# tjiangHIT/cuteSV

Hardware: NVIDIA H100
Metric: sv_signatures_clustered_per_sec (higher is better)
Workload: dtype int32

## Files before the change

### cutesv_b200/csrc/cutesv_b200.cu

```cuda
#include <cuda_runtime.h>
#include <dlfcn.h>
#include <nccl.h>
#include <stdarg.h>
#include <stdio.h>
#include <stdlib.h>
#include <string.h>

#include <algorithm>
#include <atomic>
#include <string>
#include <vector>

#include "../../include/cutesv_b200.h"
#include "core.h"
#include "devprims.cuh"
#include "host_tables.h"
#include "kernels.cuh"
#include "radix.cuh"
#include "extract.cuh"
#include "scan_core.h"

using namespace csv;

static thread_local char g_err[1024] = "";
// ... 109 lines not shown
struct LbPool {
    uint32_t* tickets = nullptr;
    const uint32_t* epoch = nullptr;
    uint32_t ord0 = 0;
    int next = 0, cap = 0;
};

struct GcWork {
    DBuf win, bin_base, bin_start, bin_fill, bin_list, iter, prim, cov_off, ovl_off, cov_fill, ovl_fill, cov_u, ovl_u, lb, words;
    DBuf r_chrom, r_start, r_end, r_id, r_prim, cov_raw, ovl_raw, cov_ded, ovl_ded, cov_flag, ovl_flag, sup_off, sup, geno;
    uint32_t n_cov = 0, n_ovl = 0;
};

struct SsWork {
    DBuf keys_a, keys_b, vals_a, vals_b, keep, tie, kchrom, order, off, hist, lb, words;
};

struct csv_ctx {
    int device = 0;
    cudaStream_t stream = nullptr;
    bool own_stream = false;
    cudaStream_t copy_stream = nullptr;
    cudaEvent_t ev_up[CSV_NTYPES + 1] = {nullptr, nullptr, nullptr, nullptr, nullptr, nullptr};
    bool up_pending[CSV_NTYPES + 1] = {false, false, false, false, false, false};
    bool up_device[CSV_NTYPES + 1] = {false, false, false, false, false, false};
    bool up_checked[CSV_NTYPES + 1] = {false, false, false, false, false, false};
    DBuf up_status;
    cudaEvent_t ev_prod = nullptr;
    cudaEvent_t ev_done = nullptr;
    bool done_pending = false;
    int n_sm = 132;
    csv_params P;
    bool have_params = false;
    int32_t n_contigs = 0;
    std::vector<int64_t> contig_len;
    std::vector<uint64_t> contig_off;
    int64_t off_pad = 0;
    std::vector<uint8_t> owned;
    DBuf d_off, d_len, d_len_eff;
    SigBuf sig[CSV_NTYPES];
    int64_t n_reads = 0;
    DBuf r_chrom, r_start, r_end, r_id, r_prim;
    int64_t n_aln = 0;
    DBuf a_chrom, a_start, a_end, a_id, a_prim, a_off, a_span;
    DBuf tickets, scan_carry, emit_cursor;
    DBuf d_epoch;
    LbPool lb;
    uint32_t epoch_host = 0;
    bool small_chain[CSV_NTYPES] = {false, false, false, false, false};
    bool prefilter_enabled = true;
    bool records_enabled = true;
    bool small_path_enabled = true;
    int64_t pair_cap_override = 0;
    DBuf d_goff[CSV_NTYPES + 1];
    Lane lanes[N_LANES];
    cudaEvent_t ev_fork = nullptr;
    cudaStream_t side_stream[2] = {nullptr, nullptr};
    cudaEvent_t ev_side_fork[2] = {nullptr, nullptr}, ev_side_join[2] = {nullptr, nullptr};
    cudaStream_t aux_stream = nullptr;
    cudaEvent_t ev_aux = nullptr;
    bool lanes_enabled = true;
    DBuf kept[CSV_NTYPES], cnt;
    uint32_t kept_cap[CSV_NTYPES] = {0, 0, 0, 0, 0};
    DBuf cand_tmp, cand, geno, names, counters;
    uint32_t cap_cand = 0, cap_names = 0;
    Counters* h_counters = nullptr;
    DBuf bin_start, bin_fill, bin_bits, win_list, win_rec, dr, has_rows, gl_table, pow_half, pairs;
    uint32_t pow_n = 0;
    bool ran = false, counts_valid = false;
    int64_t launches = 0;
    bool profiling = false;
    bool lane_marks = false;
    struct Interval { int st; cudaEvent_t a, b; int64_t bytes; };
    std::vector<Interval> ivs;
    std::vector<cudaEvent_t> ev_pool;
    size_t ev_next = 0;
    bool ivs_consumed = false;
    struct KInterval { const char* name; cudaEvent_t a, b; };
    std::vector<KInterval> kivs;
    struct KTotal { std::string name; int64_t launches; double ms; };
    std::vector<KTotal> ktotals;
    float stage_ms[CSV_ST_COUNT];
    float sort_ms = 0.f;
    int64_t sort_bytes = 0;
    int32_t sort_launches = 0;
    uint32_t last_mask = 0x1f;
    ExtractState ex;
    struct GraphKey {
        uint32_t mask; int64_t n[CSV_NTYPES]; int64_t n_reads, n_aln; csv_params P; int lanes; uint64_t alloc_epoch; uint64_t cfg_epoch;
        bool small_chain[CSV_NTYPES];
        bool up_checked[CSV_NTYPES + 1];
    };
    struct GraphSlot { bool valid = false; GraphKey key; cudaGraphExec_t exec = nullptr; int64_t launches = 0; uint64_t used = 0; };
    static constexpr int N_GRAPHS = 4;
    GraphSlot graphs[N_GRAPHS];
    GraphKey last_key;
    bool last_key_valid = false;
    bool graphs_enabled = true;
    uint64_t cfg_epoch = 1, graph_clock = 0;
    int64_t graph_replays = 0;
    struct P2PState {
        bool ready = false, failed = false;
        void* box = nullptr;
        int64_t slot_bytes = 0;
        size_t flags_off = 0;
        std::vector<void*> peer;
        DBuf d_tab;
        unsigned long long epoch = 0;
    } p2p;
    bool p2p_enabled = true;
    ncclComm_t comm = nullptr;
    int rank = 0, world = 1;
    DBuf g_send, g_recv, g_cand, g_geno, g_names, g_scratch, g_tab;
// ... 137 lines not shown
    CU(c->gl_table.ensure(gl.size() * sizeof(csv_geno)));
    CU(cudaMemcpy(c->gl_table.p, gl.data(), gl.size() * sizeof(csv_geno), cudaMemcpyHostToDevice));
    std::vector<double> ph = build_pow_half(pow_n);
    CU(c->pow_half.ensure(ph.size() * sizeof(double)));
    CU(cudaMemcpy(c->pow_half.p, ph.data(), ph.size() * sizeof(double), cudaMemcpyHostToDevice));
    c->pow_n = pow_n;
    return CSV_OK;
}

extern "C" int csv_create(int device, void* stream, csv_ctx** out) {
    if (!out) return set_err(CSV_E_INVALID, "null out");
    int n_dev = 0;
    cudaError_t e = cudaGetDeviceCount(&n_dev);
    if (e != cudaSuccess || n_dev == 0)
        return set_err(CSV_E_NODEVICE, "no CUDA device (%s): cutesv_b200 has no CPU fallback",
                       e == cudaSuccess ? "device count 0" : cudaGetErrorString(e));
    if (device < 0 || device >= n_dev) return set_err(CSV_E_INVALID, "device %d out of range (%d devices)", device, n_dev);
    cudaDeviceProp prop;
    CU(cudaGetDeviceProperties(&prop, device));
    if (prop.major != 9 || prop.minor != 0)
        return set_err(CSV_E_NODEVICE, "device %d is sm_%d%d; this library is built for sm_90a only", device, prop.major, prop.minor);
    CU(cudaSetDevice(device));
    csv_ctx* c = new csv_ctx();
    c->device = device;
    c->n_sm = prop.multiProcessorCount;
    if (stream) { c->stream = (cudaStream_t)stream; c->own_stream = false; }
    else {
        cudaError_t e2 = cudaStreamCreateWithFlags(&c->stream, cudaStreamNonBlocking);
        if (e2 != cudaSuccess) { delete c; return set_err(CSV_E_CUDA, "cudaStreamCreate: %s", cudaGetErrorString(e2)); }
        c->own_stream = true;
    }
    c->lanes[0].stream = c->stream;
    {
        cudaError_t e4 = cudaStreamCreateWithFlags(&c->copy_stream, cudaStreamNonBlocking);
        for (int i = 0; i <= CSV_NTYPES && e4 == cudaSuccess; i++) e4 = cudaEventCreateWithFlags(&c->ev_up[i], cudaEventDisableTiming);
        if (e4 == cudaSuccess) e4 = cudaEventCreateWithFlags(&c->ev_done, cudaEventDisableTiming);
        if (e4 == cudaSuccess) e4 = cudaEventCreateWithFlags(&c->ev_prod, cudaEventDisableTiming);
        if (e4 == cudaSuccess) e4 = cudaEventCreateWithFlags(&c->ev_fork, cudaEventDisableTiming);
        if (e4 == cudaSuccess) e4 = cudaStreamCreateWithFlags(&c->aux_stream, cudaStreamNonBlocking);
        if (e4 == cudaSuccess) e4 = cudaEventCreateWithFlags(&c->ev_aux, cudaEventDisableTiming);
        for (int k = 0; k < 2 && e4 == cudaSuccess; k++) {
            e4 = cudaStreamCreateWithFlags(&c->side_stream[k], cudaStreamNonBlocking);
            if (e4 == cudaSuccess) e4 = cudaEventCreateWithFlags(&c->ev_side_fork[k], cudaEventDisableTiming);
            if (e4 == cudaSuccess) e4 = cudaEventCreateWithFlags(&c->ev_side_join[k], cudaEventDisableTiming);
        }
        for (int l = 1; l < N_LANES && e4 == cudaSuccess; l++) {
            e4 = cudaStreamCreateWithFlags(&c->lanes[l].stream, cudaStreamNonBlocking);
            if (e4 == cudaSuccess) e4 = cudaEventCreateWithFlags(&c->lanes[l].ev_join, cudaEventDisableTiming);
        }
        if (e4 != cudaSuccess) { delete c; return set_err(CSV_E_CUDA, "copy stream / lanes: %s", cudaGetErrorString(e4)); }
    }
    csv_default_params(&c->P);
    if (const char* e = getenv("CUTESV_B200_PAIR_CAP")) c->pair_cap_override = atoll(e);
    if (const char* e = getenv("CUTESV_B200_NO_PREFILTER")) c->prefilter_enabled = atoi(e) == 0;
    if (const char* e = getenv("CUTESV_B200_LANES")) c->lanes_enabled = atoi(e) != 0;
    if (const char* e = getenv("CUTESV_B200_GRAPHS")) c->graphs_enabled = atoi(e) != 0;
    if (const char* e = getenv("CUTESV_B200_PDL")) c->pdl_enabled = atoi(e) != 0;
    if (const char* e = getenv("CUTESV_B200_GATHER")) c->p2p_enabled = strcmp(e, "nccl") != 0;
    if (const char* e = getenv("CUTESV_B200_RECORDS")) c->records_enabled = atoi(e) != 0;
    if (const char* e = getenv("CUTESV_B200_SMALL_PATH")) c->small_path_enabled = atoi(e) != 0;
    if (const char* e = getenv("CUTESV_B200_SMALL_CHAIN")) for (int t = 0; t < CSV_NTYPES; t++) c->small_chain[t] = atoi(e) != 0;
    for (int s = 0; s < CSV_ST_COUNT; s++) c->stage_ms[s] = 0.f;
    cudaError_t e3 = cudaMallocHost((void**)&c->h_counters, sizeof(Counters));
    if (e3 != cudaSuccess) { delete c; return set_err(CSV_E_CUDA, "cudaMallocHost: %s", cudaGetErrorString(e3)); }
    int rc = upload_tables(c, 1u << 16);
    if (rc != CSV_OK) { delete c; return rc; }
    CU(c->d_epoch.ensure(64, true));
    CU(c->emit_cursor.ensure(256, true));
    CU(c->up_status.ensure((CSV_NTYPES + 1) * 4, true));
    const int smem_warp = (CL_THREADS / 32) * WARP_M * ARENA_PER_MAX + (CL_THREADS / 32) * 40 * 8;
    CU(cudaFuncSetAttribute(k_cluster_warp<0>, cudaFuncAttributeMaxDynamicSharedMemorySize, smem_warp));
    CU(cudaFuncSetAttribute(k_cluster_warp<1>, cudaFuncAttributeMaxDynamicSharedMemorySize, smem_warp));
    CU(cudaFuncSetAttribute(k_cluster_warp<2>, cudaFuncAttributeMaxDynamicSharedMemorySize, smem_warp));
    CU(cudaFuncSetAttribute(k_cluster_warp<3>, cudaFuncAttributeMaxDynamicSharedMemorySize, smem_warp));
    CU(cudaFuncSetAttribute(k_cluster_warp<4>, cudaFuncAttributeMaxDynamicSharedMemorySize, smem_warp));
    CU(cudaFuncSetAttribute(k_cluster_warp<5>, cudaFuncAttributeMaxDynamicSharedMemorySize, smem_warp));
    CU(cudaFuncSetAttribute(k_cluster_warp<6>, cudaFuncAttributeMaxDynamicSharedMemorySize, smem_warp));
    CU(cudaFuncSetAttribute(k_cluster_warp<7>, cudaFuncAttributeMaxDynamicSharedMemorySize, smem_warp));
    CU(cudaFuncSetAttribute(k_cluster_block<0>, cudaFuncAttributeMaxDynamicSharedMemorySize, BLOCK_M * ARENA_PER_MAX));
    CU(cudaFuncSetAttribute(k_cluster_block<1>, cudaFuncAttributeMaxDynamicSharedMemorySize, BLOCK_M * ARENA_PER_MAX));
    CU(cudaFuncSetAttribute(k_cluster_block<2>, cudaFuncAttributeMaxDynamicSharedMemorySize, BLOCK_M * ARENA_PER_MAX));
    CU(cudaFuncSetAttribute(k_cluster_block<3>, cudaFuncAttributeMaxDynamicSharedMemorySize, BLOCK_M * ARENA_PER_MAX));
    CU(cudaFuncSetAttribute(k_part_filter, cudaFuncAttributeMaxDynamicSharedMemorySize, (int)pf_smem_bytes(PART_W_MAX)));
    CU(cudaFuncSetAttribute(k_part_scatter, cudaFuncAttributeMaxDynamicSharedMemorySize, (int)ps_smem_bytes()));
    *out = c;
    return CSV_OK;
}

extern "C" int csv_destroy(csv_ctx* c) {
    if (!c) return CSV_OK;
    cudaSetDevice(c->device);
    cudaStreamSynchronize(c->stream);
    for (auto& g : c->graphs) if (g.exec) cudaGraphExecDestroy(g.exec);
    if (c->comm) comm_destroy(c);
    if (c->h_gather) cudaFreeHost(c->h_gather);
    for (int l = 1; l < N_LANES; l++) {
        Lane& L = c->lanes[l];
        if (L.stream) { cudaStreamSynchronize(L.stream); cudaStreamDestroy(L.stream); }
        if (L.ev_join) cudaEventDestroy(L.ev_join);
    }
    if (c->ev_fork) cudaEventDestroy(c->ev_fork);
    if (c->aux_stream) { cudaStreamSynchronize(c->aux_stream); cudaStreamDestroy(c->aux_stream); }
    if (c->ev_aux) cudaEventDestroy(c->ev_aux);
    for (int k = 0; k < 2; k++) {
        if (c->side_stream[k]) { cudaStreamSynchronize(c->side_stream[k]); cudaStreamDestroy(c->side_stream[k]); }
        if (c->ev_side_fork[k]) cudaEventDestroy(c->ev_side_fork[k]);
// ... 668 lines not shown
    J.sv.chrom = w.u_chrom.as<int32_t>(); J.sv.a = w.u_a.as<int32_t>(); J.sv.b = w.u_b.as<int32_t>();
    J.sv.rid = w.u_rid.as<int32_t>(); J.sv.c = w.u_c.as<int32_t>();
    return run_segment_and_cluster(c, L, J, t, kslot_base);
}

static int ensure_small(Lane& L, size_t ns) {
    SmallWork& w = L.small;
    CU(w.k_rid.ensure(ns * 4)); CU(w.k_b.ensure(ns * 4)); CU(w.k_prim.ensure(ns * 8)); CU(w.perm_a.ensure(ns * 4)); CU(w.perm_b.ensure(ns * 4));
    CU(w.sel.ensure(ns * 4)); CU(w.u_chrom.ensure(ns * 4)); CU(w.u_a.ensure(ns * 4)); CU(w.u_b.ensure(ns * 4)); CU(w.u_rid.ensure(ns * 4));
    CU(w.u_c.ensure(ns * 4));
    return CSV_OK;
}
static int ensure_lane_scratch(Lane& L, size_t nm) {
    CU(L.keys_a.ensure(nm * 8)); CU(L.keys_b.ensure(nm * 8)); CU(L.vals_a.ensure(nm * 4)); CU(L.vals_b.ensure(nm * 4));
    CU(L.big_list.ensure((nm / WARP_M + 2) * 4));
    CU(L.giant_list.ensure((nm / BLOCK_M + 2) * 4));
    CU(L.giant_arena.ensure(nm * 2 * ARENA_PER_MAX + 256));
    return CSV_OK;
}

static int ensure_workspace(csv_ctx* c, uint32_t type_mask) {
    int64_t n_max = 0, n_total = 0, n_small_max = 0;
    for (int t = 0; t < CSV_NTYPES; t++) {
        if (!(type_mask >> t & 1)) continue;
        n_max = std::max(n_max, c->sig[t].n);
        n_total += c->sig[t].n;
        if (t >= CSV_INV) n_small_max = std::max(n_small_max, c->sig[t].n);
    }
    const size_t nm = (size_t)std::max<int64_t>(n_max, 1);
    int rc = ensure_lane_scratch(c->lanes[0], nm);
    if (rc) return rc;
    if (c->lanes_enabled) {
        for (int t = 1; t < CSV_NTYPES; t++) {
            const int64_t nl = (type_mask >> t & 1) ? c->sig[t].n : 0;
            if (nl == 0) continue;
            if ((rc = ensure_lane_scratch(c->lanes[t], (size_t)nl))) return rc;
            if (t >= CSV_INV && (rc = ensure_small(c->lanes[t], (size_t)nl))) return rc;
        }
    }
    CU(c->tickets.ensure(LB_ORDINALS * 4));
    CU(c->counters.ensure(sizeof(Counters)));
    if ((rc = ensure_small(c->lanes[0], (size_t)std::max<int64_t>(n_small_max, 1)))) return rc;
    uint64_t kept_total = 0;
    const int ms = std::max(1, c->P.min_support);
    for (int t = 0; t < CSV_NTYPES; t++) {
        if (!(type_mask >> t & 1)) continue;
        c->kept_cap[t] = (uint32_t)(c->sig[t].n / ms + 1);
        CU(c->kept[t].ensure((size_t)c->kept_cap[t] * 4));
        kept_total += c->kept_cap[t];
    }
    CU(c->cnt.ensure((size_t)kept_total * 4 + 4));
    const int ms_a = std::max(1, std::min(c->P.min_support, std::max(1, c->P.min_support_allele)));
    c->cap_cand = (uint32_t)(2 * (n_total / ms_a) + 16);
    c->cap_names = (uint32_t)(n_total + 16);
    CU(c->cand_tmp.ensure((size_t)c->cap_cand * sizeof(csv_cand)));
    CU(c->cand.ensure((size_t)c->cap_cand * sizeof(csv_cand)));
    CU(c->geno.ensure((size_t)c->cap_cand * sizeof(csv_geno)));
    CU(c->names.ensure((size_t)c->cap_names * 4));
    CU(c->dr.ensure((size_t)c->cap_cand * 4));
    CU(c->win_list.ensure((size_t)c->cap_cand * 2 * 4));
    CU(c->win_rec.ensure((size_t)c->cap_cand * 2 * sizeof(WinRec)));
    CU(c->has_rows.ensure((size_t)c->n_contigs + 16));
    return CSV_OK;
}

static int join_lanes(csv_ctx* c) {
    for (int l = 1; l < N_LANES; l++) {
        Lane& L = c->lanes[l];
        if (!L.used) continue;
        CU(cudaEventRecord(L.ev_join, L.stream));
        CU(cudaStreamWaitEvent(c->stream, L.ev_join, 0));
        L.used = false;
    }
    return CSV_OK;
}

static int enqueue_cluster(csv_ctx* c, uint32_t type_mask) {
    int rc;
    stage_reset_if_consumed(c);
    c->last_mask = type_mask;
    c->lb = LbPool{c->tickets.as<uint32_t>(), c->d_epoch.as<uint32_t>(), 0, 0, (int)LB_ORDINALS};
    {
        int n_lanes = 0;
        for (int t = 0; t < CSV_NTYPES; t++) n_lanes += ((type_mask >> t & 1) && c->sig[t].n > 0) ? 1 : 0;
        c->pdl_now = c->pdl_enabled && n_lanes <= 2;
    }
    LAUNCH(c, c->stream, k_begin, 1, 256, 0, c->d_epoch.as<uint32_t>(), c->tickets.as<uint32_t>(), (int)LB_ORDINALS, c->counters.as<uint32_t>(),
           (int)(sizeof(Counters) / 4), c->emit_cursor.as<unsigned long long>());
    Counters* ctr = c->counters.as<Counters>();
    uint32_t kslot_base = 0;
    const bool lanes = c->lanes_enabled;
    if (lanes) CU(cudaEventRecord(c->ev_fork, c->stream));
    for (Lane& L : c->lanes) L.used = false;
    const uint64_t total_len = c->contig_off[c->n_contigs];
    int geno_shift = 10;
    while ((total_len >> geno_shift) > (1u << 20)) geno_shift++;
    const uint32_t geno_bins = (uint32_t)(total_len >> geno_shift) + 2;
    bool aux_used = false;
    if (c->P.genotype) {
        CU(c->bin_start.ensure(((size_t)geno_bins + 1) * 4));
        CU(c->bin_fill.ensure((size_t)geno_bins * 4));
        CU(c->bin_bits.ensure(((size_t)geno_bins / 32 + 2) * 4));
        cudaStream_t rs = lanes ? c->aux_stream : c->stream;
        if (lanes) CU(cudaStreamWaitEvent(rs, c->ev_fork, 0));
        CU(cudaMemsetAsync(c->bin_start.p, 0, ((size_t)geno_bins + 1) * 4, rs));
        CU(cudaMemsetAsync(c->bin_fill.p, 0, (size_t)geno_bins * 4, rs));
        CU(cudaMemsetAsync(c->bin_bits.p, 0, ((size_t)geno_bins / 32 + 2) * 4, rs));
        CU(cudaMemsetAsync(c->has_rows.p, 0, (size_t)c->n_contigs, rs));
        if (lanes) { CU(cudaEventRecord(c->ev_aux, rs)); aux_used = true; }
    }
    for (int t = 0; t < CSV_NTYPES; t++) {
        if (!(type_mask >> t & 1) || c->sig[t].n == 0) continue;
        Lane& L = c->lanes[lanes ? t : 0];
        if (&L != &c->lanes[0] && !L.used) { CU(cudaStreamWaitEvent(L.stream, c->ev_fork, 0)); L.used = true; }
        rc = wait_upload(c, L.stream, t);
        if (!rc && c->up_checked[t]) LAUNCH(c, L.stream, k_fold_status, 1, 32, 0, c->up_status.as<uint32_t>() + t, &ctr->status);
        if (!rc) rc = (t == CSV_DEL || t == CSV_INS) ? run_indel(c, L, t, kslot_base) : run_other(c, L, t, kslot_base);
        if (rc) {
            join_lanes(c);
            if (aux_used) cudaStreamWaitEvent(c->stream, c->ev_aux, 0);
            return rc;
        }
        kslot_base += c->kept_cap[t];
    }
    rc = join_lanes(c);
    if (rc) return rc;
    if (aux_used) CU(cudaStreamWaitEvent(c->stream, c->ev_aux, 0));
    int tail_mark = -1;
    if (c->lane_marks) { kprof_begin(c, c->stream, "tail"); tail_mark = (int)c->kivs.size() - 1; }
    GenoJob G;
    memset(&G, 0, sizeof(G));
    G.cand = c->cand.as<csv_cand>(); G.geno = c->geno.as<csv_geno>(); G.names = c->names.as<int32_t>(); G.ctr = ctr;
    G.cap_cand = c->cap_cand;
    G.ct = ContigTab{c->d_off.as<uint64_t>(), c->d_len_eff.as<int64_t>(), c->n_contigs};
    G.gp = GtParams{c->P.bias_del, c->P.gt_bias_ins, c->P.bias_dup, c->P.bias_inv};
    G.shift = geno_shift;
    G.n_bins = geno_bins;
    G.bin_start = c->bin_start.as<uint32_t>(); G.bin_fill = c->bin_fill.as<uint32_t>(); G.bin_bits = c->bin_bits.as<uint32_t>();
    G.win_list = c->win_list.as<uint32_t>(); G.win_cap = c->cap_cand * 2;
    G.lin32 = (total_len + 4096) < (1ull << 32) ? 1 : 0;
    G.win_rec = c->win_rec.as<WinRec>();
    G.dr = c->dr.as<uint32_t>(); G.has_rows = c->has_rows.as<uint8_t>();
    G.gl_table = c->gl_table.as<csv_geno>();
    G.genotype = c->P.genotype;
    stage_begin(c, c->stream, CSV_ST_ORDER);
    {
        CU(c->scan_carry.ensure(64));
        uint32_t* carry = c->scan_carry.as<uint32_t>();
        uint32_t kb = 0;
        int prev = -1;
        for (int t = 0; t < CSV_NTYPES; t++) {
            if (!(type_mask >> t & 1) || c->sig[t].n == 0) continue;
            TileSync ts;
            rc = make_sync(c->lb, c->lanes[0].lb_status, c->stream, (size_t)(c->kept_cap[t] / SEL_TILE + 2), &ts);
            if (rc) return rc;
            if (prev >= 0)
                LAUNCH_PDL(c, c->stream, (k_scan_excl<8>), grid_for(c, std::max<int64_t>(c->kept_cap[t], 1), SEL_TILE, 2), SEL_THREADS, 0, c->cnt.as<uint32_t>() + kb,
                           (int64_t)c->kept_cap[t], (const uint32_t*)&ctr->n_kept[t], (const uint32_t*)(carry + prev), carry + t, ts);
            else
                LAUNCH(c, c->stream, (k_scan_excl<8>), grid_for(c, std::max<int64_t>(c->kept_cap[t], 1), SEL_TILE, 2), SEL_THREADS, 0, c->cnt.as<uint32_t>() + kb,
                       (int64_t)c->kept_cap[t], (const uint32_t*)&ctr->n_kept[t], (const uint32_t*)nullptr, carry + t, ts);
            kb += c->kept_cap[t];
            prev = t;
        }
        LAUNCH_PDL(c, c->stream, k_permute, grid_for(c, c->cap_cand, 256, 4), 256, 0, c->cand_tmp.as<csv_cand>(), c->cnt.as<uint32_t>(), ctr, c->cap_cand,
               c->cand.as<csv_cand>(), G, c->emit_cursor.as<unsigned long long>());
    }
    stage_end(c, c->stream, CSV_ST_ORDER);
    rc = wait_upload(c, c->stream, CSV_NTYPES);
    if (rc) return rc;
    if (c->up_checked[CSV_NTYPES] && c->n_reads > 0)
        LAUNCH(c, c->stream, k_fold_status, 1, 32, 0, c->up_status.as<uint32_t>() + CSV_NTYPES, &ctr->status);
    stage_begin(c, c->stream, CSV_ST_GENOTYPE);
    {
        if (c->P.genotype) {
            TileSync ts;
            rc = make_sync(c->lb, c->lanes[0].lb_status, c->stream, (size_t)((G.n_bins + 1) / (SEL_THREADS * 4) + 2), &ts);
            if (rc) return rc;
            LAUNCH_PDL(c, c->stream, (k_scan_excl<4>), grid_for(c, G.n_bins + 1, SEL_THREADS * 4, 4), SEL_THREADS, 0, G.bin_start, (int64_t)G.n_bins + 1,
                   (const uint32_t*)nullptr, (const uint32_t*)nullptr, (uint32_t*)nullptr, ts);
            LAUNCH_PDL(c, c->stream, (k_windows<1>), grid_for(c, c->cap_cand, 256, 4), 256, 0, G);
            if (c->n_reads > 0) {
                PairBuf PB;
                PB.cap = (uint32_t)std::min<int64_t>(4 * c->n_reads + (1 << 20), (int64_t)1 << 30);
                if (c->pair_cap_override > 0) PB.cap = (uint32_t)c->pair_cap_override;
                CU(c->pairs.ensure((size_t)PB.cap * (G.lin32 ? sizeof(uint4) : sizeof(uint2))));
                PB.pairs = c->pairs.as<uint2>();
                PB.pairs4 = c->pairs.as<uint4>();
                PB.count = &ctr->n_windows;
                if (G.lin32) {
                    LAUNCH_PDL(c, c->stream, (k_reads_pass<true>), std::min(grid_for(c, c->n_reads, 1024, 8), resident_grid(c, k_reads_pass<true>, 256, 0)), 256, 0, G, PB, c->r_chrom.as<int32_t>(), c->r_start.as<int32_t>(),
                           c->r_end.as<int32_t>(), c->r_id.as<int32_t>(), c->r_prim.as<uint8_t>(), c->n_reads, &ctr->status);
                    LAUNCH_PDL(c, c->stream, (k_pairs_test<true>), c->n_sm * 8, 256, 0, G, PB, c->r_chrom.as<int32_t>(), c->r_start.as<int32_t>(),
                           c->r_end.as<int32_t>(), c->r_id.as<int32_t>());
                } else {
                    LAUNCH_PDL(c, c->stream, (k_reads_pass<false>), std::min(grid_for(c, c->n_reads, 1024, 8), resident_grid(c, k_reads_pass<false>, 256, 0)), 256, 0, G, PB, c->r_chrom.as<int32_t>(), c->r_start.as<int32_t>(),
                           c->r_end.as<int32_t>(), c->r_id.as<int32_t>(), c->r_prim.as<uint8_t>(), c->n_reads, &ctr->status);
                    LAUNCH_PDL(c, c->stream, (k_pairs_test<false>), c->n_sm * 8, 256, 0, G, PB, c->r_chrom.as<int32_t>(), c->r_start.as<int32_t>(),
                           c->r_end.as<int32_t>(), c->r_id.as<int32_t>());
                }
            }
        }
        LAUNCH_PDL(c, c->stream, k_finalize, grid_for(c, c->cap_cand, 256, 4), 256, 0, G);
        if (c->P.genotype && c->n_aln > 0 && (type_mask >> CSV_TRA & 1) && c->sig[CSV_TRA].n > 0) {
            AlnView A{c->a_chrom.as<int32_t>(), c->a_start.as<int32_t>(), c->a_end.as<int32_t>(), c->a_id.as<int32_t>(), c->a_prim.as<uint8_t>(),
                      c->a_off.as<uint32_t>(), c->a_span.as<int32_t>(), c->d_len.as<int64_t>()};
            LAUNCH(c, c->stream, k_tra_genotype, c->n_sm * 8, 128, 0, G, A, c->P.bias_tra, c->P.gt_round);
        }
    }
    stage_end(c, c->stream, CSV_ST_GENOTYPE);
    if (tail_mark >= 0) CU(cudaEventRecord(c->kivs[tail_mark].b, c->stream));
    return CSV_OK;
}

static bool key_equal(const csv_ctx::GraphKey& a, const csv_ctx::GraphKey& b) { return memcmp(&a, &b, sizeof(a)) == 0; }

extern "C" int csv_cluster(csv_ctx* c, uint32_t type_mask) {
    if (!c) return set_err(CSV_E_INVALID, "null ctx");
    if (c->n_contigs == 0) return set_err(CSV_E_STATE, "csv_set_contigs has not been called");
    CU(cudaSetDevice(c->device));
    int rc = ensure_workspace(c, type_mask);
    if (rc) return rc;
    c->gathered = false;
    if (++c->epoch_host >= (1u << 21)) {
        CU(cudaDeviceSynchronize());
        CU(cudaMemset(c->d_epoch.p, 0, 64));
        for (Lane& L : c->lanes) if (L.lb_status.p) CU(cudaMemset(L.lb_status.p, 0, L.lb_status.cap));
        c->epoch_host = 1;
    }
    bool pending = false;
    for (int t = 0; t <= CSV_NTYPES; t++) {
        if (c->up_pending[t] && c->up_device[t]) { rc = wait_upload(c, c->stream, t); if (rc) return rc; }
        pending |= c->up_pending[t];
    }
    bool done = false;
    if (c->graphs_enabled && !c->profiling && !c->lane_marks && !pending) {
        csv_ctx::GraphKey key;
        memset(&key, 0, sizeof(key));
        key.mask = type_mask;
        for (int t = 0; t < CSV_NTYPES; t++) { key.n[t] = c->sig[t].n; key.small_chain[t] = c->small_chain[t]; }
        for (int t = 0; t <= CSV_NTYPES; t++) key.up_checked[t] = c->up_checked[t];
        key.n_reads = c->n_reads; key.n_aln = c->n_aln; key.P = c->P; key.lanes = c->lanes_enabled ? 1 : 0;
        key.alloc_epoch = g_alloc_epoch.load(); key.cfg_epoch = c->cfg_epoch;
        csv_ctx::GraphSlot* hit = nullptr;
        for (auto& g : c->graphs) if (g.valid && key_equal(g.key, key)) hit = &g;
        if (!hit && c->last_key_valid && key_equal(c->last_key, key)) {
            csv_ctx::GraphSlot* slot = &c->graphs[0];
            for (auto& g : c->graphs) { if (!g.valid) { slot = &g; break; } if (g.used < slot->used) slot = &g; }
            if (slot->exec) { cudaGraphExecDestroy(slot->exec); slot->exec = nullptr; }
            slot->valid = false;
            const int64_t l0 = c->launches;
            cudaGraph_t graph = nullptr;
            cudaError_t e = cudaStreamBeginCapture(c->stream, cudaStreamCaptureModeThreadLocal);
            if (e == cudaSuccess) {
                rc = enqueue_cluster(c, type_mask);
                e = cudaStreamEndCapture(c->stream, &graph);
                const int64_t n_launch = c->launches - l0;
                c->launches = l0;
                if (rc == CSV_OK && e == cudaSuccess && graph && g_alloc_epoch.load() == key.alloc_epoch &&
                    cudaGraphInstantiate(&slot->exec, graph, 0) == cudaSuccess) {
                    slot->valid = true; slot->key = key; slot->launches = n_launch;
                    hit = slot;
                } else {
                    cudaGetLastError();
                    if (rc != CSV_OK && rc != CSV_E_CUDA) { if (graph) cudaGraphDestroy(graph); return rc; }
                }
                if (graph) cudaGraphDestroy(graph);
            } else cudaGetLastError();
        }
        if (hit) {
            CU(cudaGraphLaunch(hit->exec, c->stream));
            hit->used = ++c->graph_clock;
            c->launches += hit->launches;
            c->graph_replays++;
            c->last_mask = type_mask;
            done = true;
        } else { c->last_key = key; c->last_key_valid = true; }
    }
    if (!done) {
        rc = enqueue_cluster(c, type_mask);
// ... 180 lines not shown
```

### cutesv_b200/csrc/kernels.cuh

```cuda
#pragma once
#include "core.h"
#include "devprims.cuh"
#include "radix.cuh"
#include <type_traits>

namespace csv {

static constexpr int WARP_M = 128;
static constexpr int BLOCK_M = 2048;
static constexpr int CL_THREADS = 256;

struct TypeJob {
    int svtype;
    int64_t n_host;
    const uint32_t* n_dev;
    const uint32_t* keys32;
    const uint64_t* keys64;
    IndelView iv;
    SortedView sv;
    ClusterParams cp;
    uint32_t kslot_base;
    const uint32_t* kept_start;
    uint32_t* big_list;
    uint32_t* giant_list;
// ... 862 lines not shown
        const int m = cluster_size_warp(J, s, n, WARP_M);
        if (m > WARP_M) {
            if (lane == 0) {
                const uint32_t o = atomicAdd(&ctr->n_big[J.svtype], 1u);
                if (o < J.big_cap) J.big_list[o] = k; else atomicOr(&ctr->status, ST_LIST_OVERFLOW);
            }
            continue;
        }
        n_mem += (uint32_t)m;
        run_cluster<KIND>(tm, J, s, m, pow2ceil(m), arena, red, J.kslot_base + k, E);
        __syncwarp();
    }
    if (lane == 0 && n_mem) atomicAdd(&ctr->n_members[J.svtype], n_mem);
}

__device__ __forceinline__ int64_t cluster_size_block(const TypeJob& J, int64_t s, int64_t n, int64_t* red) {
    CudaTeam<CL_THREADS> tm;
    int64_t done = 1;
    while (true) {
        const int64_t i = s + done + threadIdx.x;
        const int64_t cand = ((i >= n) || !job_linked(J, i)) ? (done + threadIdx.x) : INT64_MAX;
        const int64_t first = team_min(tm, cand, red);
        if (first != INT64_MAX) return first;
        done += CL_THREADS;
    }
}

template <int KIND>
__global__ void __launch_bounds__(CL_THREADS) k_cluster_block(TypeJob J, Emit E, Counters* ctr) {
    pdl_launch_dependents(); pdl_wait();
    extern __shared__ __align__(16) char smem[];
    __shared__ int64_t red[CL_THREADS + 8];
    const int64_t n = job_n(J);
    const uint32_t n_list = min(ctr->n_big[J.svtype], J.big_cap);
    CudaTeam<CL_THREADS> tm;
    for (uint32_t q = blockIdx.x; q < n_list; q += gridDim.x) {
        const uint32_t k = J.big_list[q];
        const int64_t s = J.kept_start[k];
        const int64_t m = cluster_size_block(J, s, n, red);
        const bool giant = m > BLOCK_M;
        const int M = pow2ceil((int)m);
        if (threadIdx.x == 0) {
            atomicAdd(&ctr->n_members[J.svtype], (uint32_t)m);
            if (giant) atomicAdd(&ctr->n_giant[J.svtype], 1u);
        }
        char* arena = giant ? (J.giant_arena + (size_t)(2 * s) * ARENA_PER_MAX) : smem;
        run_cluster<KIND>(tm, J, s, (int)m, M, arena, red, J.kslot_base + k, E);
        __syncthreads();
    }
}

struct alignas(16) WinRec { uint32_t S, E, S0, E0; int32_t names_off, names_cnt; uint32_t cand, second; };
struct GenoJob {
    csv_cand* cand;
    csv_geno* geno;
    const int32_t* names;
    const Counters* ctr;
    uint32_t cap_cand;
    ContigTab ct;
    GtParams gp;
    int shift;
    uint32_t n_bins;
    uint32_t* bin_start;
    uint32_t* bin_fill;
    uint32_t* bin_bits;
    uint32_t* win_list;
    uint32_t win_cap;
    struct WinRec* win_rec;
    int lin32;
    uint32_t* dr;
    uint8_t* has_rows;
    const csv_geno* gl_table;
    int genotype;
};

__device__ __forceinline__ uint32_t window_bin(const GenoJob& G, const csv_cand& c, int which) {
    int64_t s, e;
    window_of(c, which, G.gp, &s, &e);
    return (uint32_t)((G.ct.off[c.chrom] + (uint64_t)s) >> G.shift);
}

__global__ void k_permute(const csv_cand* __restrict__ tmp, const uint32_t* __restrict__ base, Counters* ctr, uint32_t cap,
                          csv_cand* __restrict__ out, GenoJob G, const unsigned long long* cursor) {
    pdl_launch_dependents(); pdl_wait();
    const unsigned long long cur = *cursor;
    if (blockIdx.x == 0 && threadIdx.x == 0) { ctr->n_cand = (uint32_t)(cur >> 32); ctr->n_names = (uint32_t)cur; }
    const uint32_t n = min((uint32_t)(cur >> 32), cap);
    for (uint32_t i = blockIdx.x * blockDim.x + threadIdx.x; i < n; i += gridDim.x * blockDim.x) {
        csv_cand c = tmp[i];
        const uint32_t dst = base[c.cluster] + (uint32_t)c.reserved[0];
        c.reserved[0] = 0;
        if (dst >= cap) continue;
        out[dst] = c;
        if (G.genotype) {
            const int nw = n_windows_of(c);
            for (int w = 0; w < nw; w++) {
                uint32_t b = window_bin(G, c, w);
                if (b >= G.n_bins) b = G.n_bins - 1;
                atomicAdd(&G.bin_start[b], 1u);
                atomicOr(&G.bin_bits[b >> 5], 1u << (b & 31));
            }
            G.dr[dst] = 0;
        }
    }
}

template <int PASS>
__global__ void k_windows(GenoJob G) {
    pdl_launch_dependents(); pdl_wait();
    const uint32_t n = min(G.ctr->n_cand, G.cap_cand);
    for (uint32_t i = blockIdx.x * blockDim.x + threadIdx.x; i < n; i += gridDim.x * blockDim.x) {
        const csv_cand c = G.cand[i];
        const int nw = n_windows_of(c);
        for (int w = 0; w < nw; w++) {
            uint32_t b = window_bin(G, c, w);
            if (b >= G.n_bins) b = G.n_bins - 1;
            if (PASS == 0) { atomicAdd(&G.bin_start[b], 1u); atomicOr(&G.bin_bits[b >> 5], 1u << (b & 31)); }
            else {
                const uint32_t o = G.bin_start[b] + atomicAdd(&G.bin_fill[b], 1u);
                if (o < G.win_cap) {
                    G.win_list[o] = i * 2u + (uint32_t)w;
                    if (G.lin32) {
                        const uint64_t coff = G.ct.off[c.chrom];
                        int64_t ws, we, s0 = 0, e0 = 0;
                        window_of(c, w, G.gp, &ws, &we);
                        if (w) window_of(c, 0, G.gp, &s0, &e0);
                        WinRec r;
                        r.S = (uint32_t)(coff + (uint64_t)ws); r.E = (uint32_t)(coff + (uint64_t)we);
                        r.S0 = (uint32_t)(coff + (uint64_t)s0); r.E0 = (uint32_t)(coff + (uint64_t)e0);
                        r.names_off = c.names_off; r.names_cnt = c.names_cnt; r.cand = i; r.second = (uint32_t)w;
                        *reinterpret_cast<uint4*>(&G.win_rec[o]) = *reinterpret_cast<const uint4*>(&r);
                        *(reinterpret_cast<uint4*>(&G.win_rec[o]) + 1) = *(reinterpret_cast<const uint4*>(&r) + 1);
                    }
                }
            }
        }
        if (PASS == 0) G.dr[i] = 0;
    }
}

__device__ __forceinline__ bool names_contain(const int32_t* __restrict__ names, int32_t off, int32_t n, int32_t rid) {
    const int lead = off & 3;
    const int4* q = reinterpret_cast<const int4*>(names + (off - lead));
    const int end = lead + n;
    bool found = false;
    for (int b = 0; b < end && !found; b += 8) {
        const int4 x = __ldg(q + (b >> 2));
        const int4 y = b + 4 < end ? __ldg(q + (b >> 2) + 1) : make_int4(0, 0, 0, 0);
        const int32_t v[8] = {x.x, x.y, x.z, x.w, y.x, y.y, y.z, y.w};
#pragma unroll
        for (int k = 0; k < 8; k++) found |= v[k] == rid && b + k >= lead && b + k < end;
    }
    return found;
}

__device__ __forceinline__ void test_pair(const GenoJob& G, uint64_t RS, uint64_t RE, int32_t rid, uint32_t w) {
    const uint32_t ent = G.win_list[w];
    const csv_cand c = G.cand[ent >> 1];
    const uint64_t coff = G.ct.off[c.chrom];
    int64_t s, e;
    window_of(c, (int)(ent & 1u), G.gp, &s, &e);
    if (!(RS <= coff + (uint64_t)s && RE >= coff + (uint64_t)e)) return;
    if (ent & 1u) {
        int64_t s0, e0;
        window_of(c, 0, G.gp, &s0, &e0);
        if (RS <= coff + (uint64_t)s0 && RE >= coff + (uint64_t)e0) return;
    }
    if (!names_contain(G.names, c.names_off, c.names_cnt, rid)) atomicAdd(&G.dr[ent >> 1], 1u);
}

__device__ __forceinline__ void test_pair32(const GenoJob& G, uint32_t RS, uint32_t RE, int32_t rid, uint32_t w) {
    const uint4 lo = __ldg(reinterpret_cast<const uint4*>(&G.win_rec[w])), hi = __ldg(reinterpret_cast<const uint4*>(&G.win_rec[w]) + 1);
    if (!(RS <= lo.x && RE >= lo.y)) return;
    if (hi.w && RS <= lo.z && RE >= lo.w) return;
    if (!names_contain(G.names, (int32_t)hi.x, (int32_t)hi.y, rid)) atomicAdd(&G.dr[hi.z], 1u);
}

struct PairBuf { uint2* pairs; uint4* pairs4; uint32_t cap; uint32_t* count; };

template <bool LIN32>
__global__ void __launch_bounds__(256) k_reads_pass(GenoJob G, PairBuf PB, const int32_t* __restrict__ r_chrom,
                                                    const int32_t* __restrict__ r_start, const int32_t* __restrict__ r_end,
                                                    const int32_t* __restrict__ r_id, const uint8_t* __restrict__ r_prim,
                                                    int64_t n_reads, uint32_t* status) {
    using Lin = typename std::conditional<LIN32, uint32_t, uint64_t>::type;
    pdl_launch_dependents(); pdl_wait();
    constexpr int ITEMS = 4;
    constexpr int TAB = 1024;
    constexpr Lin NO_OFF = ~(Lin)0;
    __shared__ uint32_t s_warp[17];
    __shared__ Lin s_off[TAB];
    __shared__ uint32_t s_lim[TAB];
    __shared__ uint8_t s_seen[TAB];
    const int n_tab = G.ct.n < TAB ? G.ct.n : TAB;
    for (int i = threadIdx.x; i < n_tab; i += 256) {
        s_off[i] = G.ct.len[i] < 0 ? NO_OFF : (Lin)G.ct.off[i];
        s_lim[i] = (uint32_t)(G.ct.off[i + 1] - G.ct.off[i] - 1);
        s_seen[i] = 0;
    }
    __syncthreads();
    const bool aligned = ((((uintptr_t)r_chrom) | ((uintptr_t)r_start) | ((uintptr_t)r_end) | ((uintptr_t)r_id)) & 15) == 0 &&
                         (((uintptr_t)r_prim) & 3) == 0;
    const int64_t n_tiles = (n_reads + 256 * ITEMS - 1) / (256 * ITEMS);
    int32_t ch[ITEMS], st[ITEMS], en[ITEMS], id[ITEMS];
    uint32_t pr = 0;
    auto load = [&](int64_t tile) {
        const int64_t r0 = tile * 256 * ITEMS + (int64_t)threadIdx.x * ITEMS;
        if (aligned && r0 + ITEMS <= n_reads) {
            const int4 c4 = __ldcs(reinterpret_cast<const int4*>(r_chrom + r0)), s4 = __ldcs(reinterpret_cast<const int4*>(r_start + r0));
            const int4 e4 = __ldcs(reinterpret_cast<const int4*>(r_end + r0)), i4 = __ldcs(reinterpret_cast<const int4*>(r_id + r0));
            pr = __ldcs(reinterpret_cast<const uint32_t*>(r_prim + r0));
// ... 81 lines not shown
            uint32_t x = m[j] & (0xffffffffu << (b0[j] & 31));
            if (w1 == w0) x &= 0xffffffffu >> (31 - (b1[j] & 31));
            else {
                x |= m1[j] & (0xffffffffu >> (31 - (b1[j] & 31)));
                for (uint32_t wi = w0 + 1; wi < w1 && !x; wi++) x = __ldg(&G.bin_bits[wi]);
            }
            if (x) { lo[j] = G.bin_start[b0[j]]; hi[j] = G.bin_start[b1[j] + 1]; }
        }
        uint32_t total = 0;
#pragma unroll
        for (int j = 0; j < ITEMS; j++) total += hi[j] - lo[j];
        uint32_t o = block_reserve_256(total, PB.count, s_warp, parity);
#pragma unroll
        for (int j = 0; j < ITEMS; j++) {
            const uint32_t cnt = hi[j] - lo[j];
            if (!cnt) continue;
            uint32_t k = 0;
            for (; k < cnt && (uint64_t)o + k < PB.cap; k++) {
                if (LIN32) PB.pairs4[o + k] = make_uint4((uint32_t)RS[j], (uint32_t)RE[j], (uint32_t)cid[j], lo[j] + k);
                else PB.pairs[o + k] = make_uint2((uint32_t)(r0 + j), lo[j] + k);
            }
            for (; k < cnt; k++) {
                if (LIN32) test_pair32(G, (uint32_t)RS[j], (uint32_t)RE[j], cid[j], lo[j] + k);
                else test_pair(G, RS[j], RE[j], cid[j], lo[j] + k);
            }
            o += cnt;
        }
    }
    __syncthreads();
    for (int i = threadIdx.x; i < n_tab; i += 256)
        if (s_seen[i] && !G.has_rows[i]) G.has_rows[i] = 1;
}

template <bool LIN32>
__global__ void __launch_bounds__(256) k_pairs_test(GenoJob G, PairBuf PB, const int32_t* __restrict__ r_chrom,
                                                    const int32_t* __restrict__ r_start, const int32_t* __restrict__ r_end,
                                                    const int32_t* __restrict__ r_id) {
    pdl_launch_dependents(); pdl_wait();
    const uint32_t n = min(*PB.count, PB.cap);
    for (uint32_t p = blockIdx.x * blockDim.x + threadIdx.x; p < n; p += gridDim.x * blockDim.x) {
        if (LIN32) {
            const uint4 pr = PB.pairs4[p];
            test_pair32(G, pr.x, pr.y, (int32_t)pr.z, pr.w);
        } else {
            const uint2 pr = PB.pairs[p];
            const int32_t ch = r_chrom[pr.x];
            const uint64_t off = G.ct.off[ch];
            const uint64_t RE = min(off + (uint64_t)(uint32_t)r_end[pr.x], G.ct.off[ch + 1] - 1);
            test_pair(G, off + (uint64_t)(uint32_t)r_start[pr.x], RE, r_id[pr.x], pr.y);
        }
    }
}

__global__ void k_finalize(GenoJob G) {
    pdl_launch_dependents(); pdl_wait();
    const uint32_t n = min(G.ctr->n_cand, G.cap_cand);
    for (uint32_t i = blockIdx.x * blockDim.x + threadIdx.x; i < n; i += gridDim.x * blockDim.x) {
        csv_cand c = G.cand[i];
        csv_geno g;
        g.dr = -1; g.dv = c.names_cnt; g.gt = -1; g.pl[0] = g.pl[1] = g.pl[2] = 0; g.gq = 0; g.status = 1; g.qual = 0.0;
        if (G.genotype && n_windows_of(c) > 0) {
            if (!G.has_rows[c.chrom]) {
                c.flags |= CSV_F_NO_READS;
                G.cand[i].flags = c.flags;
            } else {
                const int32_t dr = (int32_t)G.dr[i];
                g = G.gl_table[gl_index(dr, c.names_cnt)];
                g.dr = dr; g.dv = c.names_cnt;
            }
        }
        G.geno[i] = g;
    }
}

__global__ void k_aln_index(const int32_t* __restrict__ chrom, const int32_t* __restrict__ start, const int32_t* __restrict__ end, int64_t n,
                            int32_t n_contigs, int32_t* max_span, uint32_t* status) {
    for (int64_t i = (int64_t)blockIdx.x * blockDim.x + threadIdx.x; i < n; i += (int64_t)gridDim.x * blockDim.x) {
        const int32_t c = chrom[i];
        if (c < 0 || c >= n_contigs) { atomicOr(status, ST_BAD_CHROM); continue; }
        if (i > 0 && (chrom[i - 1] > c || (chrom[i - 1] == c && start[i - 1] > start[i]))) atomicOr(status, ST_UNSORTED);
        atomicMax(&max_span[c], end[i] - start[i]);
    }
}
__global__ void k_aln_off(const int32_t* __restrict__ chrom, int64_t n, int32_t n_contigs, uint32_t* __restrict__ off) {
    for (int64_t c = (int64_t)blockIdx.x * blockDim.x + threadIdx.x; c <= n_contigs; c += (int64_t)gridDim.x * blockDim.x) {
        int64_t lo = 0, hi = n;
        while (lo < hi) {
            const int64_t mid = (lo + hi) >> 1;
            if (chrom[mid] < c) lo = mid + 1; else hi = mid;
        }
        off[c] = (uint32_t)lo;
    }
}
__device__ __forceinline__ int tra_count_coverage_warp(const AlnView& A, int32_t chr, int64_t s, int64_t e, const int32_t* sup, int n_sup,
                                                       int32_t up_bound, int32_t itround, int32_t* nset, int32_t* dr, int64_t xs, int64_t xe) {
    const int lane = threadIdx.x & 31;
    const uint32_t below = (1u << lane) - 1u, upto = below | (1u << lane);
    int64_t iteration = 0, primary = 0;
    const uint32_t lo0 = A.off[chr], hi0 = A.off[chr + 1];
    uint32_t lo = lo0, hi = hi0;
    const int64_t min_start = s - (int64_t)A.max_span[chr];
    while (lo < hi) { uint32_t mid = lo + (hi - lo) / 2; if ((int64_t)A.start[mid] < min_start) lo = mid + 1; else hi = mid; }
    for (uint32_t base = lo; base < hi0; base += 32) {
        const uint32_t i = base + lane;
        const bool valid = i < hi0;
        const int64_t st = valid ? (int64_t)A.start[i] : 0, en = valid ? (int64_t)A.end[i] : 0;
        const bool before_end = valid && st < e;
        const bool fetched = before_end && en > s;
        const bool prim = fetched && A.prim[i] != 0;
        const bool spanning = prim && st < s && en > e;
        const bool fresh = spanning && !(xs <= xe && st < xs && en > xe);
        const bool is_ref = fresh && !sorted_contains(sup, n_sup, A.rid[i]);
        const uint32_t m_f = __ballot_sync(0xffffffffu, fetched), m_p = __ballot_sync(0xffffffffu, prim);
        const uint32_t m_n = __ballot_sync(0xffffffffu, fresh), m_r = __ballot_sync(0xffffffffu, is_ref);
        const int64_t it_incl = iteration + __popc(m_f & upto), pr_incl = primary + __popc(m_p & upto);
        const int32_t ns_incl = *nset + __popc(m_n & upto), dr_incl = *dr + __popc(m_r & upto);
        const bool ret_up = spanning && ns_incl >= up_bound;
        const bool ret_round = prim && it_incl >= itround;
        const uint32_t m_ret = __ballot_sync(0xffffffffu, ret_up || ret_round);
        if (m_ret) {
            const int src = __ffs(m_ret) - 1;
            int code = ret_up ? 1 : (((double)pr_incl / (double)it_incl) <= 0.2 ? 1 : -1);
            code = __shfl_sync(0xffffffffu, code, src);
            *nset = __shfl_sync(0xffffffffu, ns_incl, src);
// ... 162 lines not shown
```

Before: 17.46 billion.

## Fold candidate permutation into finalize and overlap order scan on aux stream

```diff
diff --git a/cutesv_b200/csrc/cutesv_b200.cu b/cutesv_b200/csrc/cutesv_b200.cu
--- a/cutesv_b200/csrc/cutesv_b200.cu
+++ b/cutesv_b200/csrc/cutesv_b200.cu
@@ -185,6 +185,7 @@
     bool records_enabled = true;
     bool small_path_enabled = true;
     int64_t pair_cap_override = 0;
+    int64_t cand_cap_override = 0;
     DBuf d_goff[CSV_NTYPES + 1];
     Lane lanes[N_LANES];
     cudaEvent_t ev_fork = nullptr;
@@ -192,6 +193,7 @@
     cudaEvent_t ev_side_fork[2] = {nullptr, nullptr}, ev_side_join[2] = {nullptr, nullptr};
     cudaStream_t aux_stream = nullptr;
     cudaEvent_t ev_aux = nullptr;
+    DBuf order_lb;
     bool lanes_enabled = true;
     DBuf kept[CSV_NTYPES], cnt;
     uint32_t kept_cap[CSV_NTYPES] = {0, 0, 0, 0, 0};
@@ -435,6 +437,7 @@
     }
     csv_default_params(&c->P);
     if (const char* e = getenv("CUTESV_B200_PAIR_CAP")) c->pair_cap_override = atoll(e);
+    if (const char* e = getenv("CUTESV_B200_CAND_CAP")) c->cand_cap_override = atoll(e);
     if (const char* e = getenv("CUTESV_B200_NO_PREFILTER")) c->prefilter_enabled = atoi(e) == 0;
     if (const char* e = getenv("CUTESV_B200_LANES")) c->lanes_enabled = atoi(e) != 0;
     if (const char* e = getenv("CUTESV_B200_GRAPHS")) c->graphs_enabled = atoi(e) != 0;
@@ -1209,6 +1212,7 @@
     CU(c->cnt.ensure((size_t)kept_total * 4 + 4));
     const int ms_a = std::max(1, std::min(c->P.min_support, std::max(1, c->P.min_support_allele)));
     c->cap_cand = (uint32_t)(2 * (n_total / ms_a) + 16);
+    if (c->cand_cap_override > 0) c->cap_cand = (uint32_t)std::min<int64_t>(c->cap_cand, c->cand_cap_override);
     c->cap_names = (uint32_t)(n_total + 16);
     CU(c->cand_tmp.ensure((size_t)c->cap_cand * sizeof(csv_cand)));
     CU(c->cand.ensure((size_t)c->cap_cand * sizeof(csv_cand)));
@@ -1287,6 +1291,7 @@
     if (c->lane_marks) { kprof_begin(c, c->stream, "tail"); tail_mark = (int)c->kivs.size() - 1; }
     GenoJob G;
     memset(&G, 0, sizeof(G));
+    G.tmp = c->cand_tmp.as<csv_cand>(); G.cursor = c->emit_cursor.as<unsigned long long>();
     G.cand = c->cand.as<csv_cand>(); G.geno = c->geno.as<csv_geno>(); G.names = c->names.as<int32_t>(); G.ctr = ctr;
     G.cap_cand = c->cap_cand;
     G.ct = ContigTab{c->d_off.as<uint64_t>(), c->d_len_eff.as<int64_t>(), c->n_contigs};
@@ -1300,7 +1305,16 @@
     G.dr = c->dr.as<uint32_t>(); G.has_rows = c->has_rows.as<uint8_t>();
     G.gl_table = c->gl_table.as<csv_geno>();
     G.genotype = c->P.genotype;
-    stage_begin(c, c->stream, CSV_ST_ORDER);
+    const cudaStream_t os = lanes ? c->aux_stream : c->stream;
+    if (lanes) {
+        CU(cudaEventRecord(c->ev_fork, c->stream));
+        CU(cudaStreamWaitEvent(os, c->ev_fork, 0));
+    }
+    auto join_order = [&]() -> int {
+        if (lanes) { CU(cudaEventRecord(c->ev_aux, os)); CU(cudaStreamWaitEvent(c->stream, c->ev_aux, 0)); }
+        return CSV_OK;
+    };
+    stage_begin(c, os, CSV_ST_ORDER);
     {
         CU(c->scan_carry.ensure(64));
         uint32_t* carry = c->scan_carry.as<uint32_t>();
@@ -1309,23 +1323,21 @@
         for (int t = 0; t < CSV_NTYPES; t++) {
             if (!(type_mask >> t & 1) || c->sig[t].n == 0) continue;
             TileSync ts;
-            rc = make_sync(c->lb, c->lanes[0].lb_status, c->stream, (size_t)(c->kept_cap[t] / SEL_TILE + 2), &ts);
-            if (rc) return rc;
+            rc = make_sync(c->lb, c->order_lb, os, (size_t)(c->kept_cap[t] / SEL_TILE + 2), &ts);
+            if (rc) { join_order(); return rc; }
             if (prev >= 0)
-                LAUNCH_PDL(c, c->stream, (k_scan_excl<8>), grid_for(c, std::max<int64_t>(c->kept_cap[t], 1), SEL_TILE, 2), SEL_THREADS, 0, c->cnt.as<uint32_t>() + kb,
+                LAUNCH_PDL(c, os, (k_scan_excl<8>), grid_for(c, std::max<int64_t>(c->kept_cap[t], 1), SEL_TILE, 2), SEL_THREADS, 0, c->cnt.as<uint32_t>() + kb,
                            (int64_t)c->kept_cap[t], (const uint32_t*)&ctr->n_kept[t], (const uint32_t*)(carry + prev), carry + t, ts);
             else
-                LAUNCH(c, c->stream, (k_scan_excl<8>), grid_for(c, std::max<int64_t>(c->kept_cap[t], 1), SEL_TILE, 2), SEL_THREADS, 0, c->cnt.as<uint32_t>() + kb,
+                LAUNCH(c, os, (k_scan_excl<8>), grid_for(c, std::max<int64_t>(c->kept_cap[t], 1), SEL_TILE, 2), SEL_THREADS, 0, c->cnt.as<uint32_t>() + kb,
                        (int64_t)c->kept_cap[t], (const uint32_t*)&ctr->n_kept[t], (const uint32_t*)nullptr, carry + t, ts);
             kb += c->kept_cap[t];
             prev = t;
         }
-        LAUNCH_PDL(c, c->stream, k_permute, grid_for(c, c->cap_cand, 256, 4), 256, 0, c->cand_tmp.as<csv_cand>(), c->cnt.as<uint32_t>(), ctr, c->cap_cand,
-               c->cand.as<csv_cand>(), G, c->emit_cursor.as<unsigned long long>());
-    }
-    stage_end(c, c->stream, CSV_ST_ORDER);
+    }
+    stage_end(c, os, CSV_ST_ORDER);
     rc = wait_upload(c, c->stream, CSV_NTYPES);
-    if (rc) return rc;
+    if (rc) { join_order(); return rc; }
     if (c->up_checked[CSV_NTYPES] && c->n_reads > 0)
         LAUNCH(c, c->stream, k_fold_status, 1, 32, 0, c->up_status.as<uint32_t>() + CSV_NTYPES, &ctr->status);
     stage_begin(c, c->stream, CSV_ST_GENOTYPE);
@@ -1333,9 +1345,10 @@
         if (c->P.genotype) {
             TileSync ts;
             rc = make_sync(c->lb, c->lanes[0].lb_status, c->stream, (size_t)((G.n_bins + 1) / (SEL_THREADS * 4) + 2), &ts);
-            if (rc) return rc;
+            if (rc) { join_order(); return rc; }
+            LAUNCH(c, c->stream, (k_windows<0>), grid_for(c, c->cap_cand, 256, 4), 256, 0, G);
             LAUNCH_PDL(c, c->stream, (k_scan_excl<4>), grid_for(c, G.n_bins + 1, SEL_THREADS * 4, 4), SEL_THREADS, 0, G.bin_start, (int64_t)G.n_bins + 1,
-                   (const uint32_t*)nullptr, (const uint32_t*)nullptr, (uint32_t*)nullptr, ts);
+                       (const uint32_t*)nullptr, (const uint32_t*)nullptr, (uint32_t*)nullptr, ts);
             LAUNCH_PDL(c, c->stream, (k_windows<1>), grid_for(c, c->cap_cand, 256, 4), 256, 0, G);
             if (c->n_reads > 0) {
                 PairBuf PB;
@@ -1358,7 +1371,11 @@
                 }
             }
         }
-        LAUNCH_PDL(c, c->stream, k_finalize, grid_for(c, c->cap_cand, 256, 4), 256, 0, G);
+        if ((rc = join_order())) return rc;
+        if (lanes)
+            LAUNCH(c, c->stream, k_finalize, grid_for(c, c->cap_cand, 256, 4), 256, 0, G, (const uint32_t*)c->cnt.as<uint32_t>(), ctr);
+        else
+            LAUNCH_PDL(c, c->stream, k_finalize, grid_for(c, c->cap_cand, 256, 4), 256, 0, G, (const uint32_t*)c->cnt.as<uint32_t>(), ctr);
         if (c->P.genotype && c->n_aln > 0 && (type_mask >> CSV_TRA & 1) && c->sig[CSV_TRA].n > 0) {
             AlnView A{c->a_chrom.as<int32_t>(), c->a_start.as<int32_t>(), c->a_end.as<int32_t>(), c->a_id.as<int32_t>(), c->a_prim.as<uint8_t>(),
                       c->a_off.as<uint32_t>(), c->a_span.as<int32_t>(), c->d_len.as<int64_t>()};
@@ -1383,6 +1400,7 @@
         CU(cudaDeviceSynchronize());
         CU(cudaMemset(c->d_epoch.p, 0, 64));
         for (Lane& L : c->lanes) if (L.lb_status.p) CU(cudaMemset(L.lb_status.p, 0, L.lb_status.cap));
+        if (c->order_lb.p) CU(cudaMemset(c->order_lb.p, 0, c->order_lb.cap));
         c->epoch_host = 1;
     }
     bool pending = false;
diff --git a/cutesv_b200/csrc/kernels.cuh b/cutesv_b200/csrc/kernels.cuh
--- a/cutesv_b200/csrc/kernels.cuh
+++ b/cutesv_b200/csrc/kernels.cuh
@@ -938,6 +938,8 @@
 
 struct alignas(16) WinRec { uint32_t S, E, S0, E0; int32_t names_off, names_cnt; uint32_t cand, second; };
 struct GenoJob {
+    const csv_cand* tmp;
+    const unsigned long long* cursor;
     csv_cand* cand;
     csv_geno* geno;
     const int32_t* names;
@@ -966,58 +968,31 @@
     return (uint32_t)((G.ct.off[c.chrom] + (uint64_t)s) >> G.shift);
 }
 
-__global__ void k_permute(const csv_cand* __restrict__ tmp, const uint32_t* __restrict__ base, Counters* ctr, uint32_t cap,
-                          csv_cand* __restrict__ out, GenoJob G, const unsigned long long* cursor) {
-    pdl_launch_dependents(); pdl_wait();
-    const unsigned long long cur = *cursor;
-    if (blockIdx.x == 0 && threadIdx.x == 0) { ctr->n_cand = (uint32_t)(cur >> 32); ctr->n_names = (uint32_t)cur; }
-    const uint32_t n = min((uint32_t)(cur >> 32), cap);
-    for (uint32_t i = blockIdx.x * blockDim.x + threadIdx.x; i < n; i += gridDim.x * blockDim.x) {
-        csv_cand c = tmp[i];
-        const uint32_t dst = base[c.cluster] + (uint32_t)c.reserved[0];
-        c.reserved[0] = 0;
-        if (dst >= cap) continue;
-        out[dst] = c;
-        if (G.genotype) {
-            const int nw = n_windows_of(c);
-            for (int w = 0; w < nw; w++) {
-                uint32_t b = window_bin(G, c, w);
-                if (b >= G.n_bins) b = G.n_bins - 1;
-                atomicAdd(&G.bin_start[b], 1u);
-                atomicOr(&G.bin_bits[b >> 5], 1u << (b & 31));
-            }
-            G.dr[dst] = 0;
-        }
-    }
-}
-
 template <int PASS>
 __global__ void k_windows(GenoJob G) {
     pdl_launch_dependents(); pdl_wait();
-    const uint32_t n = min(G.ctr->n_cand, G.cap_cand);
+    const uint32_t n = min((uint32_t)(*G.cursor >> 32), G.cap_cand);
     for (uint32_t i = blockIdx.x * blockDim.x + threadIdx.x; i < n; i += gridDim.x * blockDim.x) {
-        const csv_cand c = G.cand[i];
+        const csv_cand c = G.tmp[i];
         const int nw = n_windows_of(c);
         for (int w = 0; w < nw; w++) {
             uint32_t b = window_bin(G, c, w);
             if (b >= G.n_bins) b = G.n_bins - 1;
-            if (PASS == 0) { atomicAdd(&G.bin_start[b], 1u); atomicOr(&G.bin_bits[b >> 5], 1u << (b & 31)); }
-            else {
-                const uint32_t o = G.bin_start[b] + atomicAdd(&G.bin_fill[b], 1u);
-                if (o < G.win_cap) {
-                    G.win_list[o] = i * 2u + (uint32_t)w;
-                    if (G.lin32) {
-                        const uint64_t coff = G.ct.off[c.chrom];
-                        int64_t ws, we, s0 = 0, e0 = 0;
-                        window_of(c, w, G.gp, &ws, &we);
-                        if (w) window_of(c, 0, G.gp, &s0, &e0);
-                        WinRec r;
-                        r.S = (uint32_t)(coff + (uint64_t)ws); r.E = (uint32_t)(coff + (uint64_t)we);
-                        r.S0 = (uint32_t)(coff + (uint64_t)s0); r.E0 = (uint32_t)(coff + (uint64_t)e0);
-                        r.names_off = c.names_off; r.names_cnt = c.names_cnt; r.cand = i; r.second = (uint32_t)w;
-                        *reinterpret_cast<uint4*>(&G.win_rec[o]) = *reinterpret_cast<const uint4*>(&r);
-                        *(reinterpret_cast<uint4*>(&G.win_rec[o]) + 1) = *(reinterpret_cast<const uint4*>(&r) + 1);
-                    }
+            if (PASS == 0) { atomicAdd(&G.bin_start[b], 1u); atomicOr(&G.bin_bits[b >> 5], 1u << (b & 31)); continue; }
+            const uint32_t o = G.bin_start[b] + atomicAdd(&G.bin_fill[b], 1u);
+            if (o < G.win_cap) {
+                G.win_list[o] = i * 2u + (uint32_t)w;
+                if (G.lin32) {
+                    const uint64_t coff = G.ct.off[c.chrom];
+                    int64_t ws, we, s0 = 0, e0 = 0;
+                    window_of(c, w, G.gp, &ws, &we);
+                    if (w) window_of(c, 0, G.gp, &s0, &e0);
+                    WinRec r;
+                    r.S = (uint32_t)(coff + (uint64_t)ws); r.E = (uint32_t)(coff + (uint64_t)we);
+                    r.S0 = (uint32_t)(coff + (uint64_t)s0); r.E0 = (uint32_t)(coff + (uint64_t)e0);
+                    r.names_off = c.names_off; r.names_cnt = c.names_cnt; r.cand = i; r.second = (uint32_t)w;
+                    *reinterpret_cast<uint4*>(&G.win_rec[o]) = *reinterpret_cast<const uint4*>(&r);
+                    *(reinterpret_cast<uint4*>(&G.win_rec[o]) + 1) = *(reinterpret_cast<const uint4*>(&r) + 1);
                 }
             }
         }
@@ -1042,7 +1017,7 @@
 
 __device__ __forceinline__ void test_pair(const GenoJob& G, uint64_t RS, uint64_t RE, int32_t rid, uint32_t w) {
     const uint32_t ent = G.win_list[w];
-    const csv_cand c = G.cand[ent >> 1];
+    const csv_cand c = G.tmp[ent >> 1];
     const uint64_t coff = G.ct.off[c.chrom];
     int64_t s, e;
     window_of(c, (int)(ent & 1u), G.gp, &s, &e);
@@ -1230,24 +1205,36 @@
     }
 }
 
-__global__ void k_finalize(GenoJob G) {
+static_assert(sizeof(csv_cand) == 64 && sizeof(csv_geno) == 40, "k_finalize moves the records as 16 B / 8 B words");
+__global__ void k_finalize(GenoJob G, const uint32_t* __restrict__ base, Counters* ctr) {
     pdl_launch_dependents(); pdl_wait();
-    const uint32_t n = min(G.ctr->n_cand, G.cap_cand);
+    const unsigned long long cur = *G.cursor;
+    if (blockIdx.x == 0 && threadIdx.x == 0) { ctr->n_cand = (uint32_t)(cur >> 32); ctr->n_names = (uint32_t)cur; }
+    const uint32_t n = min((uint32_t)(cur >> 32), G.cap_cand);
     for (uint32_t i = blockIdx.x * blockDim.x + threadIdx.x; i < n; i += gridDim.x * blockDim.x) {
-        csv_cand c = G.cand[i];
-        csv_geno g;
+        union { csv_cand c; uint4 q[4]; } uc;
+#pragma unroll
+        for (int k = 0; k < 4; k++) uc.q[k] = __ldg(reinterpret_cast<const uint4*>(G.tmp + i) + k);
+        csv_cand& c = uc.c;
+        const uint32_t dst = base[c.cluster] + (uint32_t)c.reserved[0];
+        c.reserved[0] = 0;
+        if (dst >= G.cap_cand) continue;
+        union { csv_geno g; uint2 q[5]; } ug;
+        csv_geno& g = ug.g;
         g.dr = -1; g.dv = c.names_cnt; g.gt = -1; g.pl[0] = g.pl[1] = g.pl[2] = 0; g.gq = 0; g.status = 1; g.qual = 0.0;
         if (G.genotype && n_windows_of(c) > 0) {
             if (!G.has_rows[c.chrom]) {
                 c.flags |= CSV_F_NO_READS;
-                G.cand[i].flags = c.flags;
             } else {
                 const int32_t dr = (int32_t)G.dr[i];
                 g = G.gl_table[gl_index(dr, c.names_cnt)];
                 g.dr = dr; g.dv = c.names_cnt;
             }
         }
-        G.geno[i] = g;
+#pragma unroll
+        for (int k = 0; k < 4; k++) reinterpret_cast<uint4*>(G.cand + dst)[k] = uc.q[k];
+#pragma unroll
+        for (int k = 0; k < 5; k++) reinterpret_cast<uint2*>(G.geno + dst)[k] = ug.q[k];
     }
 }
 
```

Result: faster. 17.81 billion, median of 6 (+2.0%).
